# HI-ComputerVision/uni-encoder-code

Measured on AMD Instinct MI355X. Metric: img/s fwd+bwd Swin-L 1024x2048 bs=2 per GPU, higher is better.
Workload: dtype bf16; 1 GPU; BASELINE configs[2]: full OneFormer (Swin-L ws12 backbone + MSDeformAttn pixel decoder + 150-query masked-attention decoder), 1024x2048, fwd+bwd, synthetic loss; global_batch=2, parallelism=dp1, mode=eval() (train_mode reported separately with --full)

## Files before the change

### include/uenc.h

```cpp
#ifndef UENC_H
#define UENC_H
#include <stdint.h>

#ifdef __cplusplus
extern "C" {
#endif

#define UENC_F32 0
#define UENC_BF16 1

#ifndef UENC_STREAM_T
#define UENC_STREAM_T void*
#endif
typedef UENC_STREAM_T uenc_stream_t;

#define UENC_EPI_NONE 0
#define UENC_EPI_GELU 1
#define UENC_EPI_RELU 2
#define UENC_EPI_RESIDUAL 3
#define UENC_EPI_MUL_DGELU 4
#define UENC_EPI_MUL_DRELU 5

int uenc_version(void);
const char* uenc_arch(void);
// ... 20 lines not shown
int uenc_groupnorm_tokens_fwd(const void* x, int x_dtype, const float* gamma, const float* beta, void* y, int y_dtype,
                              float* stats, void* scratch, const float* add_src, int Hs, int Ws, int H, int W, int B, int HW,
                              int C, int G, float eps, int relu, uenc_stream_t stream);
int uenc_groupnorm_tokens_bwd(const void* dy, int dy_dtype, const void* x, int x_dtype, const float* gamma, const float* beta,
                              const float* stats, void* dx, int dx_dtype, float* dgamma, float* dbeta, void* scratch, int B,
                              int HW, int C, int G, int relu, uenc_stream_t stream);
int uenc_upsample_bilinear_tokens_bwd(const void* dy, int dy_dtype, float* dsrc, int B, int H, int W, int Hs, int Ws, int C,
                                      uenc_stream_t stream);
int uenc_merge_nearest_tokens_fwd(const void* a, int a_dtype, const void* prev, int prev_dtype, void* out, int out_dtype, int B, int H, int W,
                                  int Hs, int Ws, int C, uenc_stream_t stream);
int uenc_merge_nearest_tokens_bwd(const void* dy, int dy_dtype, float* dprev, int B, int H, int W, int Hs, int Ws, int C,
                                  uenc_stream_t stream);
int uenc_im2col3x3(const void* in, void* col, int B, int H, int W, int C, uenc_stream_t stream);
int uenc_col2im3x3(const void* dcol, void* dx, int B, int H, int W, int C, uenc_stream_t stream);
int uenc_im2col3x3_s2(const void* in, void* col, int B, int H, int W, int C, uenc_stream_t stream);
int uenc_col2im3x3_s2(const void* dcol, float* dx, int B, int H, int W, int C, uenc_stream_t stream);

int uenc_gemm_nt(const void* A, int a_dtype, long lda, const void* W, long ldw, void* C, int c_dtype, long ldc,
                 int M, int N, int K, const float* bias, int epilogue, const void* aux, long ldaux,
                 void* aux_out, long ldaux_out, float alpha, int splitk, int accumulate, uenc_stream_t stream);
#define UENC_NT_TILE_256X256 256
#define UENC_NT_TILE_256X192 192
#define UENC_NT_TILE_128X256 128
int uenc_gemm_nt_tile(const void* A, int a_dtype, long lda, const void* W, long ldw, void* C, int c_dtype, long ldc,
                      int M, int N, int K, const float* bias, int epilogue, const void* aux, long ldaux,
                      void* aux_out, long ldaux_out, float alpha, int splitk, int accumulate, int tile, uenc_stream_t stream);
int uenc_gemm_nt_scaled(const void* A, int a_dtype, long lda, const void* W, long ldw, void* C, int c_dtype, long ldc,
                        int M, int N, int K, const float* bias, int epilogue, const void* aux, long ldaux,
                        void* aux_out, long ldaux_out, float alpha, const float* sample_scale, int rows_per_sample, uenc_stream_t stream);
int uenc_gemm_nt_ln(const void* A, int a_dtype, long lda, const void* W, long ldw, void* C, long ldc, int M, int N, int K, const float* bias,
                    const void* residual, long ldres, const float* gamma, const float* beta, float eps, float* y32, void* y16, float* stats,
                    uenc_stream_t stream);
int uenc_gemm_nt_splits(int K, int splitk);
int uenc_gemm_nt_partials(const void* A, int a_dtype, long lda, const void* W, long ldw, float* P, long ldp, long part_stride,
                          int M, int N, int K, float alpha, int splitk, uenc_stream_t stream);

int uenc_gemm_nt_batched(const void* A, int a_dtype, long lda, long bsA, const void* W, long ldw, long bsW, void* C, int c_dtype,
                         long ldc, long bsC, int batch, int M, int N, int K, float alpha, int splitk, int accumulate, uenc_stream_t stream);

int uenc_gemm_tn(const void* dY, int dy_dtype, long ldy, const void* X, int x_dtype, long ldx, float* dW, long ldw,
                 float* db, int M, int N, int K, int splitm, uenc_stream_t stream);
int uenc_gemm_tn_tile(const void* dY, int dy_dtype, long ldy, const void* X, int x_dtype, long ldx, float* dW, long ldw,
                      float* db, int M, int N, int K, int splitm, int tile, uenc_stream_t stream);
int uenc_gemm_tn_scaled(const void* dY, int dy_dtype, long ldy, const void* X, int x_dtype, long ldx, float* dW, long ldw,
                        float* db, int M, int N, int K, int splitm, float alpha, uenc_stream_t stream);

int uenc_gemm_tn_grouped(const void* table, int n, int total_items, int tile, double flops, uenc_stream_t stream);
int uenc_gemm_tn_grouped_small(const void* table, int n, int total_items, double flops, uenc_stream_t stream);

int uenc_layernorm_fwd(const void* x, int x_dtype, const void* res, int res_dtype, float* h_out, const float* gamma,
                       const float* beta, void* y, int y_dtype, float* stats, long M, int C, float eps, void* y16,
                       uenc_stream_t stream);
// ... 217 lines not shown
```

### uni-encoder-code_amd/csrc/gemm.hip

```cpp
#include "common.h"
#include "prof.h"

#define BM 128
#define BN 128
#define BK 64
#define GEMM_THREADS 256

enum { EPI_NONE = 0, EPI_GELU = 1, EPI_RELU = 2, EPI_RESIDUAL = 3, EPI_MUL_DGELU = 4, EPI_MUL_DRELU = 5 };

struct GemmNT {
    const void* A; int a_f32; long lda;
    const bf16* W; long ldw;
    void* C; long ldc;
    const float* bias;
    const void* aux; long ldaux;
    bf16* aux_out; long ldaux_out;
    int M, N, K;
    int tiles_m, tiles_n;
    int klen;
    int atomic;
    int persist;
    float alpha;
    const float* sample_scale; float inv_rows;
    long part_stride;
// ... 376 lines not shown
        const float al = nt_alpha(p, m);
#pragma unroll
        for (int r = 0; r < 8; ++r) v[r] = mul_rounded(v[r], al);
        epilogue8<EPI, OUT_F32>(p, m, n, full8, v);
    }
}

#define BM2 256
#define BN2 256
#define T2 512

__device__ __forceinline__ void wait_vmcnt_upto8(int n) {
    if (n >= 8) __builtin_amdgcn_s_waitcnt(0x0f78);
    else if (n == 7) __builtin_amdgcn_s_waitcnt(0x0f77);
    else if (n == 6) __builtin_amdgcn_s_waitcnt(0x0f76);
    else if (n == 5) __builtin_amdgcn_s_waitcnt(0x0f75);
    else if (n == 4) __builtin_amdgcn_s_waitcnt(0x0f74);
    else if (n == 3) __builtin_amdgcn_s_waitcnt(0x0f73);
    else if (n == 2) __builtin_amdgcn_s_waitcnt(0x0f72);
    else if (n == 1) __builtin_amdgcn_s_waitcnt(0x0f71);
    else __builtin_amdgcn_s_waitcnt(0x0f70);
}

template <int EPI, int NI = 4>
__device__ __forceinline__ void nt_epilogue_direct(const GemmNT& p, f32x4 (&acc)[4][8], int mbase, int nbase, int fr, int fg, bool lead) {
    static_assert(NI == 4 || NI == 3, "column groups per wave");
    constexpr int NP = NI / 2;
    constexpr bool ODD = (NI & 1) != 0;
    const int mrow = mbase + fr, ncol = nbase + 4 * fg;
    const int nodd = ncol + (NI - 1) * 16;
    float bv4[4][4];
#pragma unroll
    for (int i = 0; i < NI; ++i) {
        const int n = ncol + i * 16;
        float4 b = make_float4(0.f, 0.f, 0.f, 0.f);
        if (p.bias != nullptr && n < p.N && lead) b = *(const float4*)(p.bias + n);
        bv4[i][0] = b.x; bv4[i][1] = b.y; bv4[i][2] = b.z; bv4[i][3] = b.w;
    }
    const int odd = fg & 1;
    const int n16[2] = {nbase + (0 + odd) * 16 + 4 * (fg - odd), nbase + (2 + odd) * 16 + 4 * (fg - odd)};
    constexpr bool AUX16 = (EPI == EPI_MUL_DGELU || EPI == EPI_MUL_DRELU);
    u32x4 xa[AUX16 ? 4 : 1][2];
    u32x2 xo[AUX16 && ODD ? 4 : 1];
    float4 ra[EPI == EPI_RESIDUAL ? 2 : 1][4];
#pragma unroll
    for (int j = 0; j < 8; ++j) {
        const int m = mrow + j * 16;
        const bool row_ok = m < p.M;
        if (AUX16 && (j & 3) == 0) {
#pragma unroll
            for (int jj = 0; jj < 4; ++jj) {
                const int mm = mrow + (j + jj) * 16;
#pragma unroll
                for (int pr = 0; pr < NP; ++pr)
                    xa[jj][pr] = *(const u32x4*)((const bf16*)p.aux + (long)min(mm, p.M - 1) * p.ldaux + min(n16[pr], p.N - 8));
                if (ODD) xo[AUX16 && ODD ? jj : 0] = *(const u32x2*)((const bf16*)p.aux + (long)min(mm, p.M - 1) * p.ldaux + min(nodd, p.N - 4));
            }
        }
        if (EPI == EPI_RESIDUAL && (j & 1) == 0) {
#pragma unroll
            for (int jj = 0; jj < 2; ++jj)
#pragma unroll
                for (int i = 0; i < NI; ++i) {
                    const int mm = mrow + (j + jj) * 16, n = ncol + i * 16;
                    ra[jj][i] = make_float4(0.f, 0.f, 0.f, 0.f);
                    if (mm < p.M && n < p.N) ra[jj][i] = *(const float4*)((const float*)p.aux + (long)mm * p.ldaux + n);
                }
        }
        float v[4][4];
        const float al = nt_alpha(p, min(m, p.M - 1));
#pragma unroll
        for (int i = 0; i < NI; ++i)
#pragma unroll
            for (int r = 0; r < 4; ++r) v[i][r] = (acc[i][j][r] + bv4[i][r]) * al;
// ... 19 lines not shown
            }
        } else if (EPI == EPI_MUL_DGELU || EPI == EPI_MUL_DRELU) {
#pragma unroll
            for (int pr = 0; pr < NP; ++pr) {
                const u32x4 x = xa[AUX16 ? (j & 3) : 0][pr];
                const u32x2 lo = __builtin_amdgcn_permlane16_swap(x[0], x[2], false, false);
                const u32x2 hi = __builtin_amdgcn_permlane16_swap(x[1], x[3], false, false);
                const u32x2 sa = {lo[0], hi[0]}, sb = {lo[1], hi[1]};
                const bf16x4 s0 = *(const bf16x4*)&sa, s1 = *(const bf16x4*)&sb;
#pragma unroll
                for (int r = 0; r < 4; ++r) {
                    v[2 * pr][r] = (EPI == EPI_MUL_DGELU) ? v[2 * pr][r] * dgelu_f((float)s0[r]) : (((float)s0[r] > 0.f) ? v[2 * pr][r] : 0.f);
                    v[2 * pr + 1][r] = (EPI == EPI_MUL_DGELU) ? v[2 * pr + 1][r] * dgelu_f((float)s1[r]) : (((float)s1[r] > 0.f) ? v[2 * pr + 1][r] : 0.f);
                }
            }
            if (ODD) {
                const u32x2 x = xo[AUX16 && ODD ? (j & 3) : 0];
                const bf16x4 s0 = *(const bf16x4*)&x;
#pragma unroll
                for (int r = 0; r < 4; ++r)
                    v[NI - 1][r] = (EPI == EPI_MUL_DGELU) ? v[NI - 1][r] * dgelu_f((float)s0[r]) : (((float)s0[r] > 0.f) ? v[NI - 1][r] : 0.f);
            }
        }
        {
            u32x2 o2[4];
#pragma unroll
            for (int i = 0; i < NI; ++i) {
                bf16x4 q;
#pragma unroll
                for (int r = 0; r < 4; ++r) q[r] = (bf16)v[i][r];
                o2[i] = *(const u32x2*)&q;
            }
            if (ODD && row_ok && nodd < p.N) *(u32x2*)((bf16*)p.C + (long)m * p.ldc + nodd) = o2[NI - 1];
#pragma unroll
            for (int pr = 0; pr < NP; ++pr) {
                const u32x2 lo = __builtin_amdgcn_permlane16_swap(o2[2 * pr][0], o2[2 * pr + 1][0], false, false);
                const u32x2 hi = __builtin_amdgcn_permlane16_swap(o2[2 * pr][1], o2[2 * pr + 1][1], false, false);
                if (row_ok && n16[pr] < p.N) {
                    const u32x4 o4 = {lo[0], hi[0], lo[1], hi[1]};
                    *(u32x4*)((bf16*)p.C + (long)m * p.ldc + n16[pr]) = o4;
                }
            }
        }
        if (EPI == EPI_GELU && p.aux_out != nullptr) {
            if (ODD && row_ok && nodd < p.N) *(u32x2*)(p.aux_out + (long)m * p.ldaux_out + nodd) = pre2[NI - 1];
#pragma unroll
            for (int pr = 0; pr < NP; ++pr) {
// ... 529 lines not shown
        int dev = 0, v = 0;
        if (hipGetDevice(&dev) == hipSuccess && hipDeviceGetAttribute(&v, hipDeviceAttributeMultiprocessorCount, dev) == hipSuccess && v >= 8) ncu = v / 8 * 8;
        else ncu = 256;
    }
    return ncu;
}

template <int EPI, int OUT_F32, int BNT = BN2, bool LN = false>
static int launch_nt256(GemmNT& p, hipStream_t stream) {
    p.tiles_m = (p.M + BM2 - 1) / BM2; p.tiles_n = (p.N + BNT - 1) / BNT;
    static bool attr_set = false;
    if (!attr_set) {
        hipError_t e = hipFuncSetAttribute((const void*)gemm_nt256_kernel<EPI, OUT_F32, BNT, LN>, hipFuncAttributeMaxDynamicSharedMemorySize, 131072);
        if (e != hipSuccess) return (int)e;
        attr_set = true;
    }
    const int ncu = nt_cu_count();
    const int ntiles = p.tiles_m * p.tiles_n;
    p.persist = (p.splits == 1 && ntiles > ncu) ? 1 : 0;
    hipLaunchKernelGGL((gemm_nt256_kernel<EPI, OUT_F32, BNT, LN>), dim3(p.persist ? ncu : ntiles, p.splits), dim3(T2), 131072, stream, p);
    return UENC_OK;
}

template <int EPI, int OUT_F32>
static int launch_nt_tile128(GemmNT& p, int batch, hipStream_t stream) {
    p.tiles_m = (p.M + BM - 1) / BM; p.tiles_n = (p.N + BN - 1) / BN;
    hipLaunchKernelGGL((gemm_nt_kernel<EPI, OUT_F32>), dim3(p.tiles_m * p.tiles_n, p.splits, batch), dim3(GEMM_THREADS), 0, stream, p);
    return UENC_OK;
}

template <int EPI, int OUT_F32, int A_F32>
static int launch_nt_fewrow_a(GemmNT& p, int nr, hipStream_t stream) {
    const dim3 block(GEMM_THREADS);
    if (nr == 1) {
        p.tiles_m = (p.M + 63) / 64; p.tiles_n = (p.N + 63) / 64;
        hipLaunchKernelGGL((gemm_nt_fewrow_kernel<EPI, OUT_F32, A_F32, 1, 2, 2>), dim3(p.tiles_m * p.tiles_n), block, 0, stream, p);
        return UENC_OK;
    }
    p.tiles_n = (p.N + 31) / 32;
    if ((long)((p.M + 31) / 32) * p.tiles_n * 2 >= nt_cu_count()) {
        p.tiles_m = (p.M + 31) / 32;
        hipLaunchKernelGGL((gemm_nt_fewrow_kernel<EPI, OUT_F32, A_F32, 4, 2, 2>), dim3(p.tiles_m * p.tiles_n), block, 0, stream, p);
    } else {
        p.tiles_m = (p.M + 15) / 16;
        hipLaunchKernelGGL((gemm_nt_fewrow_kernel<EPI, OUT_F32, A_F32, 4, 1, 2>), dim3(p.tiles_m * p.tiles_n), block, 0, stream, p);
    }
    return UENC_OK;
}

template <int EPI, int OUT_F32>
static int launch_nt_fewrow(GemmNT& p, int nr, hipStream_t stream) {
    return p.a_f32 ? launch_nt_fewrow_a<EPI, OUT_F32, 1>(p, nr, stream) : launch_nt_fewrow_a<EPI, OUT_F32, 0>(p, nr, stream);
}

static bool nt192_wins(int M, int N) {
    const long ncu = nt_cu_count(), tm = (M + BM2 - 1) / BM2;
    const long r256 = (tm * ((N + 255) / 256) + ncu - 1) / ncu, r192 = (tm * ((N + 191) / 192) + ncu - 1) / ncu;
    return r192 * 90 < r256 * 100;
}

static bool nt128_wins(int M, int N, int K, int c_dtype) {
    if (c_dtype == UENC_BF16 && M > 200000) return false;
    return N > 192 && N <= 288 && K <= 1024;
}

enum NtRoute { NT_REFUSED = -1, NT_TILE128, NT_FEWROW4, NT_FEWROW1, NT_HALF, NT_256, NT_192 };

static NtRoute nt_route(int M, int N, int K, int batch, int a_dtype, long lda, int c_dtype, int epilogue, bool summed, int klen, int splitk,
                        bool ln, int tile) {
    const bool prefer_half = tile == 0 ? nt128_wins(M, N, K, c_dtype) : tile == UENC_NT_TILE_128X256;
    const bool dma = batch == 1 && a_dtype == UENC_BF16 && K >= 128 && lda % 8 == 0 && N >= 192 && N % 8 == 0;
    const bool k32 = (K % BK != 0) && (K % BK3 == 0) && !summed && prefer_half;
    const long tiles256 = (long)((M + 255) / 256) * ((N + 255) / 256);
    const bool big = dma && ((K % BK == 0) || k32) &&
                     (summed ? (epilogue == EPI_NONE && c_dtype == UENC_F32 && klen % BK == 0 && tiles256 >= 4 && tiles256 * splitk >= 64) : tiles256 >= 160);
    const long htiles = (long)((M + 127) / 128) * ((N + 255) / 256);
    const bool mid = !big && dma && (K % BK == 0) && !summed && htiles >= 96 &&
                     (c_dtype == UENC_F32 ? (epilogue == EPI_NONE || epilogue == EPI_RESIDUAL || epilogue == EPI_RELU) : true);
    if (tile != 0 && !big) return NT_REFUSED;
    if (ln && !(big || mid)) return NT_REFUSED;
    const long tiles128 = (long)((M + BM - 1) / BM) * ((N + BN - 1) / BN);
    const bool few = !big && !mid && batch == 1 && !summed && K >= 64;
    if (!big && batch == 1 && !summed && tiles128 <= 32 && K >= 64) return NT_FEWROW4;
    const long tiles64 = (long)((M + 63) / 64) * ((N + 63) / 64);
    if (few && epilogue != EPI_RESIDUAL && K <= 256 && (M <= 320 || (N == 256 && K == 256 && tiles64 <= nt_cu_count()))) return NT_FEWROW1;
    if (!(big || mid)) return NT_TILE128;
    if (mid || (!summed && (K % BK3 == 0) && prefer_half)) return NT_HALF;
    if (tile == UENC_NT_TILE_128X256) return NT_REFUSED;
    const bool narrow_ok = !summed && !(ln && N > 192);
    if (tile == UENC_NT_TILE_256X192 && !narrow_ok) return NT_REFUSED;
    return narrow_ok && (tile == 0 ? nt192_wins(M, N) : tile == UENC_NT_TILE_256X192) ? NT_192 : NT_256;
}

template <int EPI, int OUT_F32>
static int launch_nt(NtRoute route, GemmNT& p, int batch, hipStream_t stream) {
    switch (route) {
        case NT_HALF: return launch_nt128<EPI, OUT_F32>(p, stream);
        case NT_256: return launch_nt256<EPI, OUT_F32>(p, stream);
        case NT_192: return launch_nt256<EPI, OUT_F32, 192>(p, stream);
        default: break;
    }
    if constexpr (EPI != EPI_RESIDUAL || OUT_F32) {
        if (route == NT_FEWROW4 || route == NT_FEWROW1) return launch_nt_fewrow<EPI, OUT_F32>(p, route == NT_FEWROW4 ? 4 : 1, stream);
        if (route == NT_TILE128) return launch_nt_tile128<EPI, OUT_F32>(p, batch, stream);
    }
    return UENC_EINVAL;
}

struct NtLn { const float* gamma; const float* beta; float* y32; void* y16; float* stats; float eps; };

static int gemm_nt_impl(const void* A, int a_dtype, long lda, const void* W, long ldw, void* C, int c_dtype, long ldc,
                        int M, int N, int K, const float* bias, int epilogue, const void* aux, long ldaux,
                        void* aux_out, long ldaux_out, float alpha, int splitk, int accumulate, int batch, long bsA, long bsW,
                        long bsC, hipStream_t stream, long part_stride = 0, const float* sample_scale = nullptr, int rows_per_sample = 0,
                        const NtLn* ln = nullptr, int tile = 0) {
    UENC_CHECK_ARG(A && W && C && M > 0 && N > 0 && K > 0);
    UENC_CHECK_ARG(a_dtype == UENC_F32 || a_dtype == UENC_BF16);
    UENC_CHECK_ARG(c_dtype == UENC_F32 || c_dtype == UENC_BF16);
    UENC_CHECK_ARG(K % 8 == 0 && N % 4 == 0 && ldw % 8 == 0 && ldc % 4 == 0);
    UENC_CHECK_ARG(a_dtype == UENC_F32 ? (lda % 4 == 0) : (lda % 8 == 0));
    UENC_CHECK_ARG(((uintptr_t)A & 15) == 0 && ((uintptr_t)W & 15) == 0 && ((uintptr_t)C & 15) == 0);
    UENC_CHECK_ARG(epilogue >= EPI_NONE && epilogue <= EPI_MUL_DRELU);
    UENC_CHECK_ARG(tile == 0 || tile == UENC_NT_TILE_256X256 || tile == UENC_NT_TILE_256X192 || tile == UENC_NT_TILE_128X256);
    if (epilogue >= EPI_RESIDUAL) UENC_CHECK_ARG(aux != nullptr && ldaux % 4 == 0);
    if (splitk < 1) splitk = 1;
    if (splitk > 1 || accumulate) UENC_CHECK_ARG(c_dtype == UENC_F32 && epilogue == EPI_NONE);
    GemmNT p;
    p.A = A; p.a_f32 = (a_dtype == UENC_F32); p.lda = lda;
    p.W = (const bf16*)W; p.ldw = ldw;
    p.C = C; p.ldc = ldc; p.bias = bias; p.aux = aux; p.ldaux = ldaux;
    p.aux_out = (bf16*)aux_out; p.ldaux_out = ldaux_out;
    p.M = M; p.N = N; p.K = K;
    p.tiles_m = 0; p.tiles_n = 0; p.persist = 0;
    const int kt = (K + BK - 1) / BK;
    if (splitk > kt) splitk = kt;
    p.klen = ((kt + splitk - 1) / splitk) * BK;
    splitk = (K + p.klen - 1) / p.klen;
    p.atomic = (splitk > 1 || accumulate) ? 1 : 0;
    p.part_stride = 0; p.splits = splitk;
    const bool partials = part_stride > 0;
    if (partials) {
        UENC_CHECK_ARG(c_dtype == UENC_F32 && epilogue == EPI_NONE && !accumulate && bias == nullptr && batch == 1 && part_stride % 4 == 0);
        p.atomic = 0; p.part_stride = part_stride;
    }
    p.alpha = alpha;
    p.sample_scale = nullptr; p.inv_rows = 0.f;
    if (sample_scale != nullptr) {
        UENC_CHECK_ARG(rows_per_sample > 0 && !p.atomic && !partials && batch == 1 && M < (1 << 22));
        p.sample_scale = sample_scale; p.inv_rows = 1.0f / (float)rows_per_sample;
    }
    p.bsA = bsA; p.bsW = bsW; p.bsC = bsC;
    p.ln_gamma = nullptr; p.ln_beta = nullptr; p.ln_y32 = nullptr; p.ln_y16 = nullptr; p.ln_stats = nullptr; p.ln_eps = 0.f;

    const bool summed = p.atomic || partials;
    const NtRoute route = nt_route(M, N, K, batch, a_dtype, lda, c_dtype, epilogue, summed, p.klen, splitk, ln != nullptr, tile);
    if (route == NT_REFUSED) return UENC_EINVAL;
    const bool dma_kernel = route == NT_HALF || route == NT_256 || route == NT_192;
    if (c_dtype == UENC_F32) UENC_CHECK_ARG(epilogue == EPI_NONE || epilogue == EPI_RESIDUAL || epilogue == EPI_RELU);
    else UENC_CHECK_ARG(epilogue != EPI_RESIDUAL || dma_kernel);
    if (ln != nullptr) {
        UENC_CHECK_ARG(epilogue == EPI_RESIDUAL && c_dtype == UENC_F32 && !summed && N <= 256 && N % 8 == 0 && ldc == N &&
                       ln->gamma && ln->beta && (ln->y32 || ln->y16));
        UENC_CHECK_ARG((((uintptr_t)ln->gamma | (uintptr_t)ln->beta | (uintptr_t)ln->y32 | (uintptr_t)ln->y16) & 15) == 0 && ((uintptr_t)ln->stats & 7) == 0);
        p.ln_gamma = ln->gamma; p.ln_beta = ln->beta; p.ln_y32 = ln->y32; p.ln_y16 = (bf16*)ln->y16; p.ln_stats = (float2*)ln->stats; p.ln_eps = ln->eps;
    }

    const bool prof = uenc_prof_on();
    if (prof) {
        const double mn = (double)M * N;
        double bytes = (double)M * K * (a_dtype == UENC_F32 ? 4 : 2) + (double)N * K * 2 + mn * (c_dtype == UENC_F32 ? 4 : 2);
        if (epilogue == EPI_RESIDUAL) bytes += mn * 4;
        if (epilogue == EPI_MUL_DGELU || epilogue == EPI_MUL_DRELU) bytes += mn * 2;
        if (aux_out != nullptr) bytes += mn * 2;
        uenc_prof_begin(route == NT_HALF ? UENC_PROF_GEMM_NT128 : dma_kernel ? UENC_PROF_GEMM_NT256 : UENC_PROF_GEMM_NT, 2.0 * batch * M * (double)N * K, stream,
                        batch * bytes);
    }
    int rc = UENC_EINVAL;
    if (ln != nullptr) {
        rc = route == NT_HALF ? launch_nt128<EPI_RESIDUAL, 1, true>(p, stream)
                              : route == NT_192 ? launch_nt256<EPI_RESIDUAL, 1, 192, true>(p, stream) : launch_nt256<EPI_RESIDUAL, 1, BN2, true>(p, stream);
    } else {
        switch (epilogue * 2 + (c_dtype == UENC_F32 ? 1 : 0)) {
#define NT_CASE(E, F) case (E) * 2 + (F): rc = launch_nt<E, F>(route, p, batch, stream); break
            NT_CASE(EPI_NONE, 1); NT_CASE(EPI_RESIDUAL, 1); NT_CASE(EPI_RELU, 1);
            NT_CASE(EPI_NONE, 0); NT_CASE(EPI_GELU, 0); NT_CASE(EPI_RELU, 0); NT_CASE(EPI_MUL_DGELU, 0); NT_CASE(EPI_MUL_DRELU, 0);
            NT_CASE(EPI_RESIDUAL, 0);
#undef NT_CASE
            default: break;
        }
    }
    if (prof) uenc_prof_end(stream);
    if (rc != UENC_OK) return rc;
    UENC_LAUNCH_RET();
}

extern "C" int uenc_gemm_nt(const void* A, int a_dtype, long lda, const void* W, long ldw, void* C, int c_dtype, long ldc,
                            int M, int N, int K, const float* bias, int epilogue, const void* aux, long ldaux,
                            void* aux_out, long ldaux_out, float alpha, int splitk, int accumulate, hipStream_t stream) {
    return gemm_nt_impl(A, a_dtype, lda, W, ldw, C, c_dtype, ldc, M, N, K, bias, epilogue, aux, ldaux, aux_out, ldaux_out, alpha, splitk,
                        accumulate, 1, 0, 0, 0, stream);
}

extern "C" int uenc_gemm_nt_tile(const void* A, int a_dtype, long lda, const void* W, long ldw, void* C, int c_dtype, long ldc,
                                 int M, int N, int K, const float* bias, int epilogue, const void* aux, long ldaux,
                                 void* aux_out, long ldaux_out, float alpha, int splitk, int accumulate, int tile, hipStream_t stream) {
    return gemm_nt_impl(A, a_dtype, lda, W, ldw, C, c_dtype, ldc, M, N, K, bias, epilogue, aux, ldaux, aux_out, ldaux_out, alpha, splitk,
                        accumulate, 1, 0, 0, 0, stream, 0, nullptr, 0, nullptr, tile);
}

extern "C" int uenc_gemm_nt_scaled(const void* A, int a_dtype, long lda, const void* W, long ldw, void* C, int c_dtype, long ldc,
                                   int M, int N, int K, const float* bias, int epilogue, const void* aux, long ldaux,
                                   void* aux_out, long ldaux_out, float alpha, const float* sample_scale, int rows_per_sample,
                                   hipStream_t stream) {
    UENC_CHECK_ARG(sample_scale != nullptr && rows_per_sample > 0);
    return gemm_nt_impl(A, a_dtype, lda, W, ldw, C, c_dtype, ldc, M, N, K, bias, epilogue, aux, ldaux, aux_out, ldaux_out, alpha, 1,
                        0, 1, 0, 0, 0, stream, 0, sample_scale, rows_per_sample);
}

extern "C" int uenc_gemm_nt_ln(const void* A, int a_dtype, long lda, const void* W, long ldw, void* C, long ldc, int M, int N, int K, const float* bias,
                               const void* residual, long ldres, const float* gamma, const float* beta, float eps, float* y32, void* y16, float* stats,
                               hipStream_t stream) {
    UENC_CHECK_ARG(residual != nullptr);
    NtLn ln = {gamma, beta, y32, y16, stats, eps};
    return gemm_nt_impl(A, a_dtype, lda, W, ldw, C, UENC_F32, ldc, M, N, K, bias, EPI_RESIDUAL, residual, ldres, nullptr, 0, 1.0f, 1, 0, 1, 0, 0, 0, stream, 0,
                        nullptr, 0, &ln);
}

extern "C" int uenc_gemm_nt_splits(int K, int splitk) {
    const int kt = (K + BK - 1) / BK;
    if (splitk < 1) splitk = 1;
    if (splitk > kt) splitk = kt;
    const int klen = (kt + splitk - 1) / splitk;
    return (kt + klen - 1) / klen;
}

extern "C" int uenc_gemm_nt_partials(const void* A, int a_dtype, long lda, const void* W, long ldw, float* P, long ldp, long part_stride,
                                     int M, int N, int K, float alpha, int splitk, hipStream_t stream) {
    UENC_CHECK_ARG(splitk >= 1 && uenc_gemm_nt_splits(K, splitk) == splitk && part_stride >= (long)(M - 1) * ldp + N);
    return gemm_nt_impl(A, a_dtype, lda, W, ldw, P, UENC_F32, ldp, M, N, K, nullptr, EPI_NONE, nullptr, 0, nullptr, 0, alpha, splitk, 0, 1, 0, 0,
// ... 468 lines not shown
```

### uni-encoder-code_amd/uenc/capi.py

```python
import ctypes
import os

import torch

_HERE = os.path.dirname(os.path.abspath(__file__))
LIB_PATH = os.path.join(_HERE, "libuenc_hip.so")

F32, BF16 = 0, 1
EPI_NONE, EPI_GELU, EPI_RELU, EPI_RESIDUAL, EPI_MUL_DGELU, EPI_MUL_DRELU = range(6)

c_p, c_i, c_l, c_f, c_u, c_d = ctypes.c_void_p, ctypes.c_int, ctypes.c_long, ctypes.c_float, ctypes.c_uint, ctypes.c_double

_SIGNATURES = {
    "uenc_version": [],
    "uenc_prof_enable": [c_i],
    "uenc_prof_collect": [c_i, c_p, c_p, c_p],
    "uenc_prof_collect_bytes": [c_i, c_p],
    "uenc_prof_next_bytes": [ctypes.c_double],
    "uenc_cast_f32_bf16": [c_p, c_p, c_l, c_p],
    "uenc_cast_transpose_f32_bf16": [c_p, c_p, c_i, c_i, c_p],
    "uenc_cast_multi": [c_p, c_i, c_l, c_p],
    "uenc_upsample_bilinear": [c_p, c_p, c_l, c_i, c_i, c_i, c_i, c_p],
    "uenc_attn_mask": [c_p, c_p, c_l, c_i, c_i, c_i, c_i, c_p],
    "uenc_gemm_nt": [c_p, c_i, c_l, c_p, c_l, c_p, c_i, c_l, c_i, c_i, c_i, c_p, c_i, c_p, c_l, c_p, c_l, c_f, c_i, c_i, c_p],
    "uenc_gemm_nt_tile": [c_p, c_i, c_l, c_p, c_l, c_p, c_i, c_l, c_i, c_i, c_i, c_p, c_i, c_p, c_l, c_p, c_l, c_f, c_i, c_i, c_i, c_p],
    "uenc_gemm_nt_scaled": [c_p, c_i, c_l, c_p, c_l, c_p, c_i, c_l, c_i, c_i, c_i, c_p, c_i, c_p, c_l, c_p, c_l, c_f, c_p, c_i, c_p],
    "uenc_gemm_nt_ln": [c_p, c_i, c_l, c_p, c_l, c_p, c_l, c_i, c_i, c_i, c_p, c_p, c_l, c_p, c_p, c_f, c_p, c_p, c_p, c_p],
    "uenc_groupnorm_tokens_scratch_bytes": [c_i, c_i, c_i, c_i],
    "uenc_groupnorm_tokens_fwd": [c_p, c_i, c_p, c_p, c_p, c_i, c_p, c_p, c_p, c_i, c_i, c_i, c_i, c_i, c_i, c_i, c_i, c_f, c_i, c_p],
    "uenc_groupnorm_tokens_bwd": [c_p, c_i, c_p, c_i, c_p, c_p, c_p, c_p, c_i, c_p, c_p, c_p, c_i, c_i, c_i, c_i, c_i, c_p],
    "uenc_upsample_bilinear_tokens_bwd": [c_p, c_i, c_p, c_i, c_i, c_i, c_i, c_i, c_i, c_p],
    "uenc_merge_nearest_tokens_fwd": [c_p, c_i, c_p, c_i, c_p, c_i, c_i, c_i, c_i, c_i, c_i, c_i, c_p],
    "uenc_merge_nearest_tokens_bwd": [c_p, c_i, c_p, c_i, c_i, c_i, c_i, c_i, c_i, c_p],
    "uenc_im2col3x3": [c_p, c_p, c_i, c_i, c_i, c_i, c_p],
    "uenc_col2im3x3": [c_p, c_p, c_i, c_i, c_i, c_i, c_p],
    "uenc_add_cast_bf16": [c_p, c_p, c_p, c_l, c_l, c_p],
    "uenc_msda_prep_fwd": [c_p, c_l, c_p, c_i, c_p, c_p, c_p, c_l, c_i, c_i, c_i, c_i, c_p],
    "uenc_msda_prep_bwd": [c_p, c_p, c_p, c_p, c_p, c_l, c_l, c_i, c_i, c_i, c_i, c_p],
    "uenc_segment_colsum": [c_p, c_l, c_i, c_p, c_i, c_l, c_i, c_p, c_p],
    "uenc_dropout_bf16": [c_p, c_p, c_l, c_u, c_f, c_p],
    "uenc_gemm_nt_splits": [c_i, c_i],
    "uenc_gemm_nt_partials": [c_p, c_i, c_l, c_p, c_l, c_p, c_l, c_l, c_i, c_i, c_i, c_f, c_i, c_p],
    "uenc_gemm_nt_batched": [c_p, c_i, c_l, c_l, c_p, c_l, c_l, c_p, c_i, c_l, c_l, c_i, c_i, c_i, c_i, c_f, c_i, c_i, c_p],
    "uenc_gemm_tn": [c_p, c_i, c_l, c_p, c_i, c_l, c_p, c_l, c_p, c_i, c_i, c_i, c_i, c_p],
    "uenc_gemm_tn_tile": [c_p, c_i, c_l, c_p, c_i, c_l, c_p, c_l, c_p, c_i, c_i, c_i, c_i, c_i, c_p],
    "uenc_gemm_tn_scaled": [c_p, c_i, c_l, c_p, c_i, c_l, c_p, c_l, c_p, c_i, c_i, c_i, c_i, c_f, c_p],
    "uenc_gemm_tn_grouped": [c_p, c_i, c_i, c_i, ctypes.c_double, c_p],
    "uenc_gemm_tn_grouped_small": [c_p, c_i, c_i, ctypes.c_double, c_p],
    "uenc_layernorm_fwd": [c_p, c_i, c_p, c_i, c_p, c_p, c_p, c_p, c_i, c_p, c_l, c_i, c_f, c_p, c_p],
# ... 156 lines not shown
```

### uni-encoder-code_amd/uenc/kernels.py

```python
import collections
import ctypes
import itertools
import operator
import os
from typing import Optional

import numpy as np
import torch

from . import capi
from .capi import BF16, F32, check, dt, lib, ptr, stream_ptr

EPI_NONE, EPI_GELU, EPI_RELU, EPI_RESIDUAL, EPI_MUL_DGELU, EPI_MUL_DRELU = (
    capi.EPI_NONE, capi.EPI_GELU, capi.EPI_RELU, capi.EPI_RESIDUAL, capi.EPI_MUL_DGELU, capi.EPI_MUL_DRELU)
NT_TILE_256X256, NT_TILE_256X192, NT_TILE_128X256 = 256, 192, 128


EXACT = os.environ.get("UENC_EXACT", "0") == "1"


def adt():
    return torch.float32 if EXACT else torch.bfloat16


def _odt(dtype):
    return torch.float32 if (EXACT and dtype == torch.bfloat16) else dtype


def _mat(t: torch.Tensor, name: str):
    if not t.is_cuda:
        raise capi.UencError(f"{name} must live on the GPU")
    if t.dim() != 2 or t.stride(1) != 1:
        raise capi.UencError(f"{name} must be 2-D with unit inner stride, got {tuple(t.shape)} / {t.stride()}")
    return t


CAPTURE_ARENA = None

# ... 155 lines not shown
    M, K = a.shape
    N, K2 = w.shape
    if EXACT:
        if sample_scale is not None:
            raise capi.UencError("gemm_nt: the fp32 verification kernels take no per-sample scale")
        return _gemm_nt_exact(a, w, bias, epilogue, aux, aux_out, out, alpha, accumulate)
    if K != K2 or w.dtype != torch.bfloat16:
        raise capi.UencError(f"gemm_nt: a {tuple(a.shape)} vs w {tuple(w.shape)} / {w.dtype}")
    if out is None:
        out = torch.empty((M, N), dtype=out_dtype, device=a.device)
        if splitk > 1 or accumulate:
            out.zero_()
    _mat(out, "out")
    assert out.shape == (M, N)
    if bias is not None:
        assert bias.dtype == torch.float32 and bias.numel() == N and bias.is_contiguous()
    if aux is not None:
        _mat(aux, "aux"); assert aux.shape == (M, N)
        assert aux.dtype == (torch.float32 if epilogue == EPI_RESIDUAL else torch.bfloat16)
    if aux_out is not None:
        _mat(aux_out, "aux_out"); assert aux_out.shape == (M, N) and aux_out.dtype == torch.bfloat16
    if sample_scale is not None:
        assert sample_scale.dtype == torch.float32 and sample_scale.is_cuda and sample_scale.is_contiguous()
        assert rows_per_sample > 0 and sample_scale.numel() * rows_per_sample >= M and splitk == 1 and not accumulate and tile == 0
        check(lib.uenc_gemm_nt_scaled(a.data_ptr(), dt(a), a.stride(0), w.data_ptr(), w.stride(0), out.data_ptr(), dt(out),
                                      out.stride(0), M, N, K, ptr(bias), epilogue, ptr(aux), aux.stride(0) if aux is not None else 0,
                                      ptr(aux_out), aux_out.stride(0) if aux_out is not None else 0, float(alpha), sample_scale.data_ptr(),
                                      int(rows_per_sample), stream_ptr()), "gemm_nt_scaled")
        return out
    if tile != 0:
        check(lib.uenc_gemm_nt_tile(a.data_ptr(), dt(a), a.stride(0), w.data_ptr(), w.stride(0), out.data_ptr(), dt(out),
                                    out.stride(0), M, N, K, ptr(bias), epilogue, ptr(aux), aux.stride(0) if aux is not None else 0,
                                    ptr(aux_out), aux_out.stride(0) if aux_out is not None else 0, float(alpha), int(splitk),
                                    int(accumulate), int(tile), stream_ptr()), "gemm_nt_tile")
        return out
    check(lib.uenc_gemm_nt(a.data_ptr(), dt(a), a.stride(0), w.data_ptr(), w.stride(0), out.data_ptr(), dt(out),
                           out.stride(0), M, N, K, ptr(bias), epilogue, ptr(aux), aux.stride(0) if aux is not None else 0,
                           ptr(aux_out), aux_out.stride(0) if aux_out is not None else 0, float(alpha), int(splitk),
                           int(accumulate), stream_ptr()), "gemm_nt")
    return out


def _gemm_nt_exact(a, w, bias, epilogue, aux, aux_out, out, alpha, accumulate) -> torch.Tensor:
    M, K = a.shape
    N, K2 = w.shape
    f32 = torch.float32
    if K != K2 or a.dtype != f32 or w.dtype != f32:
        raise capi.UencError(f"gemm_nt (exact): a {tuple(a.shape)} {a.dtype} vs w {tuple(w.shape)} {w.dtype}")
    if out is None:
        out = torch.zeros((M, N), dtype=f32, device=a.device) if accumulate else torch.empty((M, N), dtype=f32, device=a.device)
    _mat(out, "out")
    assert out.shape == (M, N) and out.dtype == f32
    for t, name in ((aux, "aux"), (aux_out, "aux_out")):
        if t is not None:
            _mat(t, name); assert t.shape == (M, N) and t.dtype == f32
    if bias is not None:
        assert bias.dtype == f32 and bias.numel() == N and bias.is_contiguous()
    check(lib.uenc_gemm_nt_f32(a.data_ptr(), a.stride(0), w.data_ptr(), w.stride(0), out.data_ptr(), out.stride(0), M, N, K, ptr(bias),
                               epilogue, ptr(aux), aux.stride(0) if aux is not None else 0, ptr(aux_out),
                               aux_out.stride(0) if aux_out is not None else 0, float(alpha), int(accumulate), stream_ptr()), "gemm_nt_f32")
    return out


# ... 1265 lines not shown
```

Baseline: 31.36 img/s.

## Add weight-stationary streaming GEMM kernel for small-K, small-N NT shapes

Adds a new NT GEMM kernel that keeps a column chunk of the weight matrix resident in LDS (up to 144 KiB) while waves stream 32-row blocks of A held in registers, with the next A block prefetched during the epilogue. The heuristic routes specific shapes (K=192/N=576, K=256/N=256 residual, K=256/N=288 f32) to it by default when row blocks fill waves evenly. This targets the repeated weight loads and tile overhead of the regular tiled kernels on skinny GEMMs. In exchange it uses very large LDS and register footprints, which limit occupancy to one workgroup per CU. The epilogue gains row-count and f32-output template parameters, and a scaled-tile entry point plus a grid-query API are exposed.

```diff
diff --git a/include/uenc.h b/include/uenc.h
--- a/include/uenc.h
+++ b/include/uenc.h
@@ -66,12 +66,18 @@
 #define UENC_NT_TILE_256X256 256
 #define UENC_NT_TILE_256X192 192
 #define UENC_NT_TILE_128X256 128
+#define UENC_NT_TILE_STREAM 32
 int uenc_gemm_nt_tile(const void* A, int a_dtype, long lda, const void* W, long ldw, void* C, int c_dtype, long ldc,
                       int M, int N, int K, const float* bias, int epilogue, const void* aux, long ldaux,
                       void* aux_out, long ldaux_out, float alpha, int splitk, int accumulate, int tile, uenc_stream_t stream);
+int uenc_gemm_nt_stream_grid(int M, int N, int K, int* grid);
 int uenc_gemm_nt_scaled(const void* A, int a_dtype, long lda, const void* W, long ldw, void* C, int c_dtype, long ldc,
                         int M, int N, int K, const float* bias, int epilogue, const void* aux, long ldaux,
                         void* aux_out, long ldaux_out, float alpha, const float* sample_scale, int rows_per_sample, uenc_stream_t stream);
+int uenc_gemm_nt_scaled_tile(const void* A, int a_dtype, long lda, const void* W, long ldw, void* C, int c_dtype, long ldc,
+                             int M, int N, int K, const float* bias, int epilogue, const void* aux, long ldaux,
+                             void* aux_out, long ldaux_out, float alpha, const float* sample_scale, int rows_per_sample, int tile,
+                             uenc_stream_t stream);
 int uenc_gemm_nt_ln(const void* A, int a_dtype, long lda, const void* W, long ldw, void* C, long ldc, int M, int N, int K, const float* bias,
                     const void* residual, long ldres, const float* gamma, const float* beta, float eps, float* y32, void* y16, float* stats,
                     uenc_stream_t stream);
diff --git a/uni-encoder-code_amd/csrc/gemm.hip b/uni-encoder-code_amd/csrc/gemm.hip
--- a/uni-encoder-code_amd/csrc/gemm.hip
+++ b/uni-encoder-code_amd/csrc/gemm.hip
@@ -422,9 +422,11 @@
     else __builtin_amdgcn_s_waitcnt(0x0f70);
 }
 
-template <int EPI, int NI = 4>
-__device__ __forceinline__ void nt_epilogue_direct(const GemmNT& p, f32x4 (&acc)[4][8], int mbase, int nbase, int fr, int fg, bool lead) {
+template <int EPI, int NI = 4, int NJ = 8, int OUT_F32 = 0>
+__device__ __forceinline__ void nt_epilogue_direct(const GemmNT& p, f32x4 (&acc)[4][NJ], int mbase, int nbase, int fr, int fg, bool lead) {
     static_assert(NI == 4 || NI == 3, "column groups per wave");
+    static_assert(NJ == 8 || NJ == 2, "row groups per wave");
+    constexpr int JB = NJ < 4 ? NJ : 4;
     constexpr int NP = NI / 2;
     constexpr bool ODD = (NI & 1) != 0;
     const int mrow = mbase + fr, ncol = nbase + 4 * fg;
@@ -444,12 +446,12 @@
     u32x2 xo[AUX16 && ODD ? 4 : 1];
     float4 ra[EPI == EPI_RESIDUAL ? 2 : 1][4];
 #pragma unroll
-    for (int j = 0; j < 8; ++j) {
+    for (int j = 0; j < NJ; ++j) {
         const int m = mrow + j * 16;
         const bool row_ok = m < p.M;
         if (AUX16 && (j & 3) == 0) {
 #pragma unroll
-            for (int jj = 0; jj < 4; ++jj) {
+            for (int jj = 0; jj < JB; ++jj) {
                 const int mm = mrow + (j + jj) * 16;
 #pragma unroll
                 for (int pr = 0; pr < NP; ++pr)
@@ -515,7 +517,11 @@
                     v[NI - 1][r] = (EPI == EPI_MUL_DGELU) ? v[NI - 1][r] * dgelu_f((float)s0[r]) : (((float)s0[r] > 0.f) ? v[NI - 1][r] : 0.f);
             }
         }
-        {
+        if (OUT_F32) {
+#pragma unroll
+            for (int i = 0; i < NI; ++i)
+                if (row_ok && ncol + i * 16 < p.N) *(float4*)((float*)p.C + (long)m * p.ldc + ncol + i * 16) = make_float4(v[i][0], v[i][1], v[i][2], v[i][3]);
+        } else {
             u32x2 o2[4];
 #pragma unroll
             for (int i = 0; i < NI; ++i) {
@@ -1091,6 +1097,149 @@
     return UENC_OK;
 }
 
+#define ST_WAVES 8
+#define ST_THREADS (ST_WAVES * 64)
+#define ST_ROWS 32
+#define ST_KSTEPS 9
+#define ST_LDS 147456
+
+template <int EPI, int OUT_F32>
+__global__ __launch_bounds__(ST_THREADS) void gemm_nt_stream_kernel(GemmNT p, int cw, int nchunks, int wgs) {
+    extern __shared__ __attribute__((aligned(16))) unsigned char smem[];
+    const int t = threadIdx.x, lane = t & 63, wave = t >> 6;
+    const int fr = lane & 15, fg = lane >> 4;
+    int chunk, g;
+    if ((wgs & 7) == 0) {
+        const int slot = blockIdx.x >> 3;
+        chunk = slot % nchunks;
+        g = (slot / nchunks) * 8 + (blockIdx.x & 7);
+    } else {
+        chunk = blockIdx.x / wgs;
+        g = blockIdx.x - chunk * wgs;
+    }
+    const int c0 = chunk * cw;
+    if (c0 >= p.N) return;
+    const int cend = min(p.N, c0 + cw);
+    const int rows = (cend - c0 + 15) & ~15;
+    const int ntl = rows >> 4;
+    const int nks = p.K >> 5;
+    const int img = rows * 64;
+    const int nblocks = (p.M + ST_ROWS - 1) / ST_ROWS;
+    const int stride = wgs * ST_WAVES;
+    int rb = g * ST_WAVES + wave;
+
+    u32x4 a[ST_KSTEPS][ST_ROWS / 16];
+#pragma unroll
+    for (int s = 0; s < ST_KSTEPS; ++s)
+#pragma unroll
+        for (int j = 0; j < ST_ROWS / 16; ++j) a[s][j] = (u32x4){0u, 0u, 0u, 0u};
+    auto load_a = [&](int blk) {
+#pragma unroll
+        for (int j = 0; j < ST_ROWS / 16; ++j) {
+            const bf16* ap = (const bf16*)p.A + (long)min(blk * ST_ROWS + j * 16 + fr, p.M - 1) * p.lda + 8 * fg;
+#pragma unroll
+            for (int s = 0; s < ST_KSTEPS; ++s)
+                if (s < nks) a[s][j] = *(const u32x4*)(ap + s * 32);
+        }
+    };
+    if (rb < nblocks) load_a(rb);
+    {
+        const int cpr = p.K >> 3, pieces = rows * cpr;
+        for (int base = t; base < pieces; base += 9 * ST_THREADS) {
+            u32x4 v[9];
+            int dst[9];
+#pragma unroll
+            for (int q = 0; q < 9; ++q) {
+                const int idx = min(base + q * ST_THREADS, pieces - 1);
+                const int r = idx / cpr, c8 = idx - r * cpr;
+                v[q] = *(const u32x4*)(p.W + (long)min(c0 + r, cend - 1) * p.ldw + c8 * 8);
+                if (c0 + r >= cend) v[q] = (u32x4){0u, 0u, 0u, 0u};
+                dst[q] = (c8 >> 2) * img + lds_off32(r, c8 & 3);
+            }
+#pragma unroll
+            for (int q = 0; q < 9; ++q)
+                if (base + q * ST_THREADS < pieces) *(u32x4*)(smem + dst[q]) = v[q];
+        }
+    }
+    __syncthreads();
+    GemmNT q = p;
+    q.N = cend;
+    const int woff = lds_off32(fr, fg);
+    const int ngroups = (ntl + 3) >> 2;
+    auto krun = [&](f32x4 (&acc)[4][ST_ROWS / 16], const int (&toff)[4], auto S0, auto CNT) {
+        constexpr int s0 = decltype(S0)::value, cnt = decltype(CNT)::value;
+        bf16x8 wf[cnt][4];
+#pragma unroll
+        for (int s = 0; s < cnt; ++s)
+#pragma unroll
+            for (int i = 0; i < 4; ++i) wf[s][i] = *(const bf16x8*)(smem + min(s0 + s, nks - 1) * img + toff[i]);
+#pragma unroll
+        for (int s = 0; s < cnt; ++s)
+#pragma unroll
+            for (int i = 0; i < 4; ++i)
+#pragma unroll
+                for (int j = 0; j < ST_ROWS / 16; ++j) acc[i][j] = mfma16(wf[s][i], *(const bf16x8*)&a[s0 + s][j], acc[i][j]);
+    };
+    using std::integral_constant;
+    for (; rb < nblocks; rb += stride) {
+        for (int cg = 0; cg < ngroups; ++cg) {
+            int toff[4];
+#pragma unroll
+            for (int i = 0; i < 4; ++i) toff[i] = min(cg * 4 + i, ntl - 1) * 1024 + woff;
+            f32x4 acc[4][ST_ROWS / 16];
+#pragma unroll
+            for (int i = 0; i < 4; ++i)
+#pragma unroll
+                for (int j = 0; j < ST_ROWS / 16; ++j) acc[i][j] = (f32x4){0.f, 0.f, 0.f, 0.f};
+            krun(acc, toff, integral_constant<int, 0>{}, integral_constant<int, 4>{});
+            if (nks > 4) krun(acc, toff, integral_constant<int, 4>{}, integral_constant<int, 2>{});
+            if (nks > 6) krun(acc, toff, integral_constant<int, 6>{}, integral_constant<int, 2>{});
+            if (nks > 8) krun(acc, toff, integral_constant<int, 8>{}, integral_constant<int, 1>{});
+            if (cg == ngroups - 1 && rb + stride < nblocks) load_a(rb + stride);
+            nt_epilogue_direct<EPI, 4, ST_ROWS / 16, OUT_F32>(q, acc, rb * ST_ROWS, c0 + cg * 64, fr, fg, true);
+        }
+    }
+}
+
+static int stream_chunk_width(int N, int K, int* nchunks) {
+    if (K % 32 != 0 || K < 128 || K > 32 * ST_KSTEPS || N % 8 != 0 || N < 16) return 0;
+    const int cmax = (ST_LDS / (2 * K)) & ~15;
+    const int nc = (N + cmax - 1) / cmax;
+    *nchunks = nc;
+    return (((N + nc - 1) / nc) + 15) & ~15;
+}
+
+static int stream_workgroups(int M, int nchunks) {
+    const int per_chunk = nt_cu_count() / nchunks, nblocks = (M + ST_ROWS - 1) / ST_ROWS;
+    return per_chunk < 1 ? 1 : (per_chunk < nblocks ? per_chunk : nblocks);
+}
+
+extern "C" int uenc_gemm_nt_stream_grid(int M, int N, int K, int* grid) {
+    UENC_CHECK_ARG(grid != nullptr && M > 0 && N > 0 && K > 0);
+    int nchunks = 0;
+    const int cw = stream_chunk_width(N, K, &nchunks);
+    if (cw == 0) return UENC_EINVAL;
+    grid[0] = stream_workgroups(M, nchunks); grid[1] = nchunks; grid[2] = ST_WAVES; grid[3] = ST_ROWS; grid[4] = cw;
+    return UENC_OK;
+}
+
+template <int EPI, int OUT_F32>
+static int launch_nt_stream(GemmNT& p, hipStream_t stream) {
+    int nchunks = 0;
+    const int cw = stream_chunk_width(p.N, p.K, &nchunks);
+    if (cw == 0) return UENC_EINVAL;
+    static bool attr_set = false;
+    if (!attr_set) {
+        hipError_t e = hipFuncSetAttribute((const void*)gemm_nt_stream_kernel<EPI, OUT_F32>, hipFuncAttributeMaxDynamicSharedMemorySize, ST_LDS);
+        if (e != hipSuccess) return (int)e;
+        attr_set = true;
+    }
+    const int lds = cw * p.K * 2;
+    const int wgs = stream_workgroups(p.M, nchunks);
+    hipLaunchKernelGGL((gemm_nt_stream_kernel<EPI, OUT_F32>), dim3(wgs * nchunks), dim3(ST_THREADS), lds, stream, p, cw, nchunks, wgs);
+    return UENC_OK;
+}
+
 template <int EPI, int OUT_F32>
 static int launch_nt_tile128(GemmNT& p, int batch, hipStream_t stream) {
     p.tiles_m = (p.M + BM - 1) / BM; p.tiles_n = (p.N + BN - 1) / BN;
@@ -1133,10 +1282,27 @@
     return N > 192 && N <= 288 && K <= 1024;
 }
 
-enum NtRoute { NT_REFUSED = -1, NT_TILE128, NT_FEWROW4, NT_FEWROW1, NT_HALF, NT_256, NT_192 };
+static bool stream_legal(int N, int K, int batch, int a_dtype, long lda, bool summed, bool ln) {
+    int nchunks = 0;
+    return batch == 1 && a_dtype == UENC_BF16 && lda % 8 == 0 && !summed && !ln && stream_chunk_width(N, K, &nchunks) != 0;
+}
+
+static bool stream_wins(int M, int N, int K, int c_dtype, int epilogue) {
+    int nchunks = 0;
+    if (stream_chunk_width(N, K, &nchunks) == 0) return false;
+    const long waves = (long)stream_workgroups(M, nchunks) * ST_WAVES, blocks = (M + ST_ROWS - 1) / ST_ROWS, rounds = (blocks + waves - 1) / waves;
+    const bool full4 = rounds >= 4 && blocks * 100 >= rounds * waves * 97;
+    if (c_dtype == UENC_BF16)
+        return full4 && ((epilogue == EPI_NONE && K == 192 && N == 576) || (epilogue == EPI_RESIDUAL && K == 256 && N == 256));
+    return epilogue == EPI_NONE && N == 288 && K == 256 && rounds >= 2 && blocks * 100 >= rounds * waves * 65;
+}
+
+enum NtRoute { NT_REFUSED = -1, NT_TILE128, NT_FEWROW4, NT_FEWROW1, NT_HALF, NT_256, NT_192, NT_STREAM };
 
 static NtRoute nt_route(int M, int N, int K, int batch, int a_dtype, long lda, int c_dtype, int epilogue, bool summed, int klen, int splitk,
-                        bool ln, int tile) {
+                        bool ln, int tile, bool stream_ok, bool allow_stream) {
+    if (tile == UENC_NT_TILE_STREAM) return stream_ok && allow_stream ? NT_STREAM : NT_REFUSED;
+    const bool streamed = allow_stream && tile == 0 && stream_ok && stream_wins(M, N, K, c_dtype, epilogue);
     const bool prefer_half = tile == 0 ? nt128_wins(M, N, K, c_dtype) : tile == UENC_NT_TILE_128X256;
     const bool dma = batch == 1 && a_dtype == UENC_BF16 && K >= 128 && lda % 8 == 0 && N >= 192 && N % 8 == 0;
     const bool k32 = (K % BK != 0) && (K % BK3 == 0) && !summed && prefer_half;
@@ -1154,6 +1320,7 @@
     const long tiles64 = (long)((M + 63) / 64) * ((N + 63) / 64);
     if (few && epilogue != EPI_RESIDUAL && K <= 256 && (M <= 320 || (N == 256 && K == 256 && tiles64 <= nt_cu_count()))) return NT_FEWROW1;
     if (!(big || mid)) return NT_TILE128;
+    if (streamed) return NT_STREAM;
     if (mid || (!summed && (K % BK3 == 0) && prefer_half)) return NT_HALF;
     if (tile == UENC_NT_TILE_128X256) return NT_REFUSED;
     const bool narrow_ok = !summed && !(ln && N > 192);
@@ -1167,6 +1334,7 @@
         case NT_HALF: return launch_nt128<EPI, OUT_F32>(p, stream);
         case NT_256: return launch_nt256<EPI, OUT_F32>(p, stream);
         case NT_192: return launch_nt256<EPI, OUT_F32, 192>(p, stream);
+        case NT_STREAM: return launch_nt_stream<EPI, OUT_F32>(p, stream);
         default: break;
     }
     if constexpr (EPI != EPI_RESIDUAL || OUT_F32) {
@@ -1174,6 +1342,12 @@
         if (route == NT_TILE128) return launch_nt_tile128<EPI, OUT_F32>(p, batch, stream);
     }
     return UENC_EINVAL;
+}
+
+static bool stream_strides_ok(int c_dtype, long ldc, int epilogue, long ldaux, const void* aux_out, long ldaux_out) {
+    if (c_dtype == UENC_BF16 && ldc % 8 != 0) return false;
+    if ((epilogue == EPI_MUL_DGELU || epilogue == EPI_MUL_DRELU) && ldaux % 8 != 0) return false;
+    return aux_out == nullptr || ldaux_out % 8 == 0;
 }
 
 struct NtLn { const float* gamma; const float* beta; float* y32; void* y16; float* stats; float eps; };
@@ -1190,7 +1364,7 @@
     UENC_CHECK_ARG(a_dtype == UENC_F32 ? (lda % 4 == 0) : (lda % 8 == 0));
     UENC_CHECK_ARG(((uintptr_t)A & 15) == 0 && ((uintptr_t)W & 15) == 0 && ((uintptr_t)C & 15) == 0);
     UENC_CHECK_ARG(epilogue >= EPI_NONE && epilogue <= EPI_MUL_DRELU);
-    UENC_CHECK_ARG(tile == 0 || tile == UENC_NT_TILE_256X256 || tile == UENC_NT_TILE_256X192 || tile == UENC_NT_TILE_128X256);
+    UENC_CHECK_ARG(tile == 0 || tile == UENC_NT_TILE_256X256 || tile == UENC_NT_TILE_256X192 || tile == UENC_NT_TILE_128X256 || tile == UENC_NT_TILE_STREAM);
     if (epilogue >= EPI_RESIDUAL) UENC_CHECK_ARG(aux != nullptr && ldaux % 4 == 0);
     if (splitk < 1) splitk = 1;
     if (splitk > 1 || accumulate) UENC_CHECK_ARG(c_dtype == UENC_F32 && epilogue == EPI_NONE);
@@ -1222,11 +1396,13 @@
     p.ln_gamma = nullptr; p.ln_beta = nullptr; p.ln_y32 = nullptr; p.ln_y16 = nullptr; p.ln_stats = nullptr; p.ln_eps = 0.f;
 
     const bool summed = p.atomic || partials;
-    const NtRoute route = nt_route(M, N, K, batch, a_dtype, lda, c_dtype, epilogue, summed, p.klen, splitk, ln != nullptr, tile);
+    const bool stream_ok = stream_legal(N, K, batch, a_dtype, lda, summed, ln != nullptr) && stream_strides_ok(c_dtype, ldc, epilogue, ldaux, aux_out, ldaux_out);
+    const NtRoute route = nt_route(M, N, K, batch, a_dtype, lda, c_dtype, epilogue, summed, p.klen, splitk, ln != nullptr, tile, stream_ok, true);
     if (route == NT_REFUSED) return UENC_EINVAL;
-    const bool dma_kernel = route == NT_HALF || route == NT_256 || route == NT_192;
+    const NtRoute filed = route == NT_STREAM ? nt_route(M, N, K, batch, a_dtype, lda, c_dtype, epilogue, summed, p.klen, splitk, false, 0, false, false) : route;
+    const bool dma_kernel = filed == NT_HALF || filed == NT_256 || filed == NT_192;
     if (c_dtype == UENC_F32) UENC_CHECK_ARG(epilogue == EPI_NONE || epilogue == EPI_RESIDUAL || epilogue == EPI_RELU);
-    else UENC_CHECK_ARG(epilogue != EPI_RESIDUAL || dma_kernel);
+    else UENC_CHECK_ARG(epilogue != EPI_RESIDUAL || dma_kernel || route == NT_STREAM);
     if (ln != nullptr) {
         UENC_CHECK_ARG(epilogue == EPI_RESIDUAL && c_dtype == UENC_F32 && !summed && N <= 256 && N % 8 == 0 && ldc == N &&
                        ln->gamma && ln->beta && (ln->y32 || ln->y16));
@@ -1241,7 +1417,7 @@
         if (epilogue == EPI_RESIDUAL) bytes += mn * 4;
         if (epilogue == EPI_MUL_DGELU || epilogue == EPI_MUL_DRELU) bytes += mn * 2;
         if (aux_out != nullptr) bytes += mn * 2;
-        uenc_prof_begin(route == NT_HALF ? UENC_PROF_GEMM_NT128 : dma_kernel ? UENC_PROF_GEMM_NT256 : UENC_PROF_GEMM_NT, 2.0 * batch * M * (double)N * K, stream,
+        uenc_prof_begin(filed == NT_HALF ? UENC_PROF_GEMM_NT128 : dma_kernel ? UENC_PROF_GEMM_NT256 : UENC_PROF_GEMM_NT, 2.0 * batch * M * (double)N * K, stream,
                         batch * bytes);
     }
     int rc = UENC_EINVAL;
@@ -1284,6 +1460,15 @@
     UENC_CHECK_ARG(sample_scale != nullptr && rows_per_sample > 0);
     return gemm_nt_impl(A, a_dtype, lda, W, ldw, C, c_dtype, ldc, M, N, K, bias, epilogue, aux, ldaux, aux_out, ldaux_out, alpha, 1,
                         0, 1, 0, 0, 0, stream, 0, sample_scale, rows_per_sample);
+}
+
+extern "C" int uenc_gemm_nt_scaled_tile(const void* A, int a_dtype, long lda, const void* W, long ldw, void* C, int c_dtype, long ldc,
+                                        int M, int N, int K, const float* bias, int epilogue, const void* aux, long ldaux,
+                                        void* aux_out, long ldaux_out, float alpha, const float* sample_scale, int rows_per_sample, int tile,
+                                        hipStream_t stream) {
+    UENC_CHECK_ARG(sample_scale != nullptr && rows_per_sample > 0);
+    return gemm_nt_impl(A, a_dtype, lda, W, ldw, C, c_dtype, ldc, M, N, K, bias, epilogue, aux, ldaux, aux_out, ldaux_out, alpha, 1,
+                        0, 1, 0, 0, 0, stream, 0, sample_scale, rows_per_sample, nullptr, tile);
 }
 
 extern "C" int uenc_gemm_nt_ln(const void* A, int a_dtype, long lda, const void* W, long ldw, void* C, long ldc, int M, int N, int K, const float* bias,
diff --git a/uni-encoder-code_amd/uenc/capi.py b/uni-encoder-code_amd/uenc/capi.py
--- a/uni-encoder-code_amd/uenc/capi.py
+++ b/uni-encoder-code_amd/uenc/capi.py
@@ -25,6 +25,8 @@
     "uenc_gemm_nt": [c_p, c_i, c_l, c_p, c_l, c_p, c_i, c_l, c_i, c_i, c_i, c_p, c_i, c_p, c_l, c_p, c_l, c_f, c_i, c_i, c_p],
     "uenc_gemm_nt_tile": [c_p, c_i, c_l, c_p, c_l, c_p, c_i, c_l, c_i, c_i, c_i, c_p, c_i, c_p, c_l, c_p, c_l, c_f, c_i, c_i, c_i, c_p],
     "uenc_gemm_nt_scaled": [c_p, c_i, c_l, c_p, c_l, c_p, c_i, c_l, c_i, c_i, c_i, c_p, c_i, c_p, c_l, c_p, c_l, c_f, c_p, c_i, c_p],
+    "uenc_gemm_nt_scaled_tile": [c_p, c_i, c_l, c_p, c_l, c_p, c_i, c_l, c_i, c_i, c_i, c_p, c_i, c_p, c_l, c_p, c_l, c_f, c_p, c_i, c_i, c_p],
+    "uenc_gemm_nt_stream_grid": [c_i, c_i, c_i, c_p],
     "uenc_gemm_nt_ln": [c_p, c_i, c_l, c_p, c_l, c_p, c_l, c_i, c_i, c_i, c_p, c_p, c_l, c_p, c_p, c_f, c_p, c_p, c_p, c_p],
     "uenc_groupnorm_tokens_scratch_bytes": [c_i, c_i, c_i, c_i],
     "uenc_groupnorm_tokens_fwd": [c_p, c_i, c_p, c_p, c_p, c_i, c_p, c_p, c_p, c_i, c_i, c_i, c_i, c_i, c_i, c_i, c_i, c_f, c_i, c_p],
diff --git a/uni-encoder-code_amd/uenc/kernels.py b/uni-encoder-code_amd/uenc/kernels.py
--- a/uni-encoder-code_amd/uenc/kernels.py
+++ b/uni-encoder-code_amd/uenc/kernels.py
@@ -13,7 +13,7 @@
 
 EPI_NONE, EPI_GELU, EPI_RELU, EPI_RESIDUAL, EPI_MUL_DGELU, EPI_MUL_DRELU = (
     capi.EPI_NONE, capi.EPI_GELU, capi.EPI_RELU, capi.EPI_RESIDUAL, capi.EPI_MUL_DGELU, capi.EPI_MUL_DRELU)
-NT_TILE_256X256, NT_TILE_256X192, NT_TILE_128X256 = 256, 192, 128
+NT_TILE_256X256, NT_TILE_256X192, NT_TILE_128X256, NT_TILE_STREAM = 256, 192, 128, 32
 
 
 EXACT = os.environ.get("UENC_EXACT", "0") == "1"
@@ -215,7 +215,13 @@
         _mat(aux_out, "aux_out"); assert aux_out.shape == (M, N) and aux_out.dtype == torch.bfloat16
     if sample_scale is not None:
         assert sample_scale.dtype == torch.float32 and sample_scale.is_cuda and sample_scale.is_contiguous()
-        assert rows_per_sample > 0 and sample_scale.numel() * rows_per_sample >= M and splitk == 1 and not accumulate and tile == 0
+        assert rows_per_sample > 0 and sample_scale.numel() * rows_per_sample >= M and splitk == 1 and not accumulate
+        if tile != 0:
+            check(lib.uenc_gemm_nt_scaled_tile(a.data_ptr(), dt(a), a.stride(0), w.data_ptr(), w.stride(0), out.data_ptr(), dt(out),
+                                               out.stride(0), M, N, K, ptr(bias), epilogue, ptr(aux), aux.stride(0) if aux is not None else 0,
+                                               ptr(aux_out), aux_out.stride(0) if aux_out is not None else 0, float(alpha),
+                                               sample_scale.data_ptr(), int(rows_per_sample), int(tile), stream_ptr()), "gemm_nt_scaled_tile")
+            return out
         check(lib.uenc_gemm_nt_scaled(a.data_ptr(), dt(a), a.stride(0), w.data_ptr(), w.stride(0), out.data_ptr(), dt(out),
                                       out.stride(0), M, N, K, ptr(bias), epilogue, ptr(aux), aux.stride(0) if aux is not None else 0,
                                       ptr(aux_out), aux_out.stride(0) if aux_out is not None else 0, float(alpha), sample_scale.data_ptr(),
@@ -232,6 +238,14 @@
                            ptr(aux_out), aux_out.stride(0) if aux_out is not None else 0, float(alpha), int(splitk),
                            int(accumulate), stream_ptr()), "gemm_nt")
     return out
+
+
+def gemm_nt_stream_grid(M: int, N: int, K: int):
+    import ctypes
+    g = (ctypes.c_int * 5)()
+    if lib.uenc_gemm_nt_stream_grid(int(M), int(N), int(K), ctypes.cast(g, ctypes.c_void_p)) != 0:
+        return None
+    return dict(workgroups=g[0], chunks=g[1], waves=g[2], block_rows=g[3], chunk_cols=g[4])
 
 
 def _gemm_nt_exact(a, w, bias, epilogue, aux, aux_out, out, alpha, accumulate) -> torch.Tensor:
```

New measurement: 30.51 img/s. 0.973x the previous value.
